# bharatlytics/faceRecognition_InfrenceEngine

Measured on AMD Instinct MI355X. Metric: faces/sec end-to-end @1080p, higher is better.
Workload: dtype f16

## Files before the change

### facerecognition_infrenceengine_amd/_lib.py

```python
import ctypes as C
import struct
import os
import threading

_HERE = os.path.dirname(os.path.abspath(__file__))
LIB_PATH = os.path.join(_HERE, "csrc", "libfrhip.so")

_lock = threading.Lock()
_lib = None
ABI_VERSION = 106


class FrError(RuntimeError):
    pass


class ConvArgs(C.Structure):
    _fields_ = [("x", C.c_void_p), ("w", C.c_void_p), ("y", C.c_void_p),
                ("bias", C.c_void_p), ("slope", C.c_void_p), ("residual", C.c_void_p),
                ("out_f32_partial", C.c_void_p),
                ("B", C.c_int), ("H", C.c_int), ("W", C.c_int), ("Cin", C.c_int), ("Cout", C.c_int),
                ("KH", C.c_int), ("KW", C.c_int), ("stride", C.c_int), ("pad", C.c_int),
                ("Ho", C.c_int), ("Wo", C.c_int), ("bias_mode", C.c_int), ("splitk", C.c_int),
                ("x2", C.c_void_p), ("C2", C.c_int)]
# ... 6 lines not shown
class ConvF8Args(C.Structure):
    _fields_ = [("x8", C.c_void_p), ("w8", C.c_void_p), ("y16", C.c_void_p), ("y8", C.c_void_p),
                ("oscale", C.c_void_p), ("bias", C.c_void_p), ("slope", C.c_void_p), ("residual", C.c_void_p),
                ("B", C.c_int), ("H", C.c_int), ("W", C.c_int), ("Cin", C.c_int), ("Cout", C.c_int),
                ("bias_mode", C.c_int), ("y8_mul", C.c_float), ("y8_sub", C.c_void_p)]


class RolePtr(C.c_void_p):
    role = None


class PnetLevel(C.Structure):
    _fields_ = [("x1", C.c_void_p), ("head", C.c_void_p), ("workspace", C.c_void_p), ("H1", C.c_int), ("W1", C.c_int),
                ("scale", C.c_float), ("boxes", C.c_void_p), ("scores", C.c_void_p), ("regs", C.c_void_p),
                ("counts", C.c_void_p), ("block_counts", C.c_void_p),
                ("x1s", C.c_void_p), ("hs", C.c_int), ("ws", C.c_int), ("f16", C.c_int)]


class FrameRef(C.Structure):
    _fields_ = [("data", C.c_void_p), ("H", C.c_int32), ("W", C.c_int32), ("nh", C.c_int32), ("nw", C.c_int32),
                ("reserved", C.c_int32 * 2)]


class Call(C.Structure):
    _fields_ = [("fn", C.c_int32), ("nargs", C.c_int32), ("a", C.c_uint64 * 22)]


_P, _I, _L, _F, _Z = C.c_void_p, C.c_int, C.c_int64, C.c_float, C.c_size_t
SEQ_FN = {"fr_dconv_mfma_f32": 1, "fr_pnet23_split_f16": 2, "fr_pnet_candidates": 3, "fr_sort_nms": 4, "fr_box_refine": 5,
          "fr_crop_conv1_f32": 6, "fr_stage_select": 7}

SIGNATURES = {
    "fr_version": (_I, []),
    "fr_last_error_string": (C.c_char_p, []),
    "fr_device_count": (_I, []),
    "fr_l2norm_rows_f32": (_I, [_P, _P, _I, _I, _P]),
    "fr_gallery_match_workspace": (_Z, [_I, _L]),
    "fr_gallery_match_f32": (_I, [_P, _P, _I, _L, _I, _L, _P, _P, _P, _Z, _P, _I, _P]),
    "fr_gallery_match_view_f32": (_I, [_P, _P, _P, _I, _L, _I, _P, _P, _P, _Z, _P]),
    "fr_gallery_topk_workspace": (_Z, [_I, _L, _I]),
    "fr_gallery_topk_f32": (_I, [_P, _P, _I, _L, _I, _I, _L, _P, _P, _P, _Z, _P, _I, _P]),
    "fr_gallery_topk_view_f32": (_I, [_P, _P, _P, _I, _L, _I, _I, _P, _P, _P, _Z, _P]),
    "fr_gallery_update_rows_f32": (_I, [_P, _P, _P, _I, _I, _I, _P]),
    "fr_gallery_match_f16_workspace": (_Z, [_I, _L]),
    "fr_gallery_match_f16": (_I, [_P, _P, _P, _I, _L, _I, _L, _P, _P, _P, _Z, _P, _I, _P]),
    "fr_gallery_match_f8_workspace": (_Z, [_I, _L]),
    "fr_gallery_match_f8": (_I, [_P, _P, _P, _I, _L, _I, _L, _P, _P, _P, _Z, _P, _I, _P]),
    "fr_gallery_update_rows_shadow": (_I, [_P, _P, _I, _P, _P, _I, _I, _I, _P]),
    "fr_gallery_match_view_f16_workspace": (_Z, [_I, _L]),
    "fr_gallery_match_view_f16": (_I, [_P, _P, _P, _P, _I, _L, _L, _I, _P, _P, _P, _Z, _P]),
    "fr_gallery_match_view_f8_workspace": (_Z, [_I, _L]),
    "fr_gallery_match_view_f8": (_I, [_P, _P, _P, _P, _I, _L, _L, _I, _P, _P, _P, _Z, _P]),
    "fr_gallery_topk_f16_workspace": (_Z, [_I, _L, _I]),
    "fr_gallery_topk_f16": (_I, [_P, _P, _P, _I, _L, _I, _I, _L, _P, _P, _P, _P, _P, _Z, _P, _I, _P]),
    "fr_gallery_topk_view_f16_workspace": (_Z, [_I, _L, _I]),
    "fr_gallery_topk_view_f16": (_I, [_P, _P, _P, _P, _I, _L, _L, _I, _I, _P, _P, _P, _P, _P, _Z, _P]),
    "fr_gallery_topk_view_masked_f32": (_I, [_P, _P, _P, _I, _L, _I, _I, _P, _P, _P, _Z, _P, _P]),
    "fr_gallery_match_grouped_workspace": (_Z, [_I, _L]),
    "fr_gallery_match_grouped_f32": (_I, [_P, _P, _P, _P, _P, _I, _I, _L, _L, _I, _P, _P, _P, _Z, _P, _I, _P]),
    "fr_gallery_topk_grouped_workspace": (_Z, [_I, _L, _I]),
    "fr_gallery_topk_grouped_f32": (_I, [_P, _P, _P, _P, _P, _I, _I, _L, _L, _I, _I, _P, _P, _P, _Z, _P, _I, _P]),
    "fr_gallery_gmax_update": (_I, [_P, _P, _L, _I, _P, _P]),
    "fr_f32_to_f8": (_I, [_P, _P, _L, _P]),
    "fr_f32_to_f16": (_I, [_P, _P, _L, _P]),
    "fr_match_decide": (_I, [_P, _P, _I, _F, _F, _P, _P]),
    "fr_match_pack_candidates": (_I, [_P, _P, _I, _P, _P]),
    "fr_match_reduce_shards": (_I, [_P, _I, _I, _I, _I, _P, _P, _P]),
    "fr_match_reduce_shards_topk": (_I, [_P, _I, _I, _I, _I, _I, _P, _P, _P]),
    "fr_exchange_pack_queries": (_I, [_P, _I, _I, _I, _P, _P]),
    "fr_exchange_counts": (_I, [_P, _I, _I, _I, _P, _P]),
    "fr_gallery_first_above_f32": (_I, [_P, _P, _I, _L, _I, _F, _I, _L, _P, _P, _P, _Z, _P]),
    "fr_cosine_matrix_f32": (_I, [_P, _P, _I, _I, _I, _P, _P]),
    "fr_mean_rows_f32": (_I, [_P, _I, _I, _P, _P]),
    "fr_unknown_assign_batch_f32": (_I, [_P, _P, _I, _I, _F, _P, _P, _P, _I, _I, _P, _P, _P, _P]),
    "fr_gallery_first_above_blocked_f32": (_I, [_P, _P, _P, _P, _I, _L, _I, _F, _I, _L, _P, _P, _P, _Z, _P]),
    "fr_enrol_batch_workspace": (_Z, [_I, _L]),
    "fr_enrol_batch_f32": (_I, [_P, _P, _I, _P, _P, _I, _P, _I, _I, _I, _P, _P, _L, _F, _F, _P, _P, _P, _P, _P, _P, _P, _P,
                                _Z, _P]),
    "fr_gallery_pairs_workspace": (_Z, [_L, _L]),
    "fr_gallery_pairs_above_f16": (_I, [_P, _P, _L, _I, _F, _I, _L, _I, _P, _P, _P, _P, _Z, _P]),
    "fr_conv_nhwc_f16": (_I, [C.POINTER(ConvArgs), _P]),
    "fr_conv_sequence": (_I, [C.POINTER(ConvStep), _I, _P]),
    "fr_conv_inblock_f16": (_I, [C.POINTER(ConvArgs), _P]),
    "fr_conv_nhwc_f8": (_I, [C.POINTER(ConvF8Args), _P]),
    "fr_quantize_f16_f8": (_I, [_P, _P, _L, _F, _P]),
    "fr_quantize_f16_f8_centred": (_I, [_P, _P, _L, _I, _P, _F, _P]),
    "fr_gptq_round_e4m3": (_I, [_P, _P, _P, _P, _I, _I, _P]),
    "fr_conv_stage14_weight_bytes": (_Z, [_I]),
    "fr_conv_stage14_pack": (_I, [_P, _P, _P]),
    "fr_conv_stage14_f16": (_I, [_P, _P, _P, _P, _I, _I, _P]),
    "fr_conv_walk64_weight_bytes": (_Z, [_I]),
    "fr_conv_walk64_pack": (_I, [_P, _P, _I, _P]),
    "fr_conv_walk64_f16": (_I, [_P, _P, _P, _P, _I, _P, _P, _I, _I, _I, _P]),
    "fr_conv_stage28_weight_bytes": (_Z, [_I]),
    "fr_conv_stage28_pack": (_I, [_P, _P, _P]),
    "fr_conv_stage28_f16": (_I, [_P, _P, _P, _P, _I, _I, _P]),
    "fr_conv_stage14_f8_weight_bytes": (_Z, [_I]),
    "fr_conv_stage14_f8_param_floats": (_Z, []),
    "fr_conv_stage14_f8_pack": (_I, [_P, _P, _P]),
    "fr_conv_stage14_f8": (_I, [_P, _P, _P, _P, _P, _I, _I, _P]),
    "fr_conv_splitk_epilogue": (_I, [_P, _I, _I, _I, _I, _I, _P, _I, _P, _P, _P, _P]),
    "fr_fc_reduce_l2norm": (_I, [_P, _I, _I, _I, _P, _P, _P, _P]),
    "fr_warp_affine_5pt": (_I, [_P, _I, _I, _I, _P, _P, _P, _I, _I, _P, _P, _P, _P]),
    "fr_warp_affine_5pt_slots": (_I, [_P, _I, _I, _I, _P, _P, _I, _I, _P, _P]),
    "fr_warp_affine_5pt_refs": (_I, [_P, _I, _P, _P, _P, _I, _I, _P, _P, _P, _P]),
    "fr_warp_affine_5pt_slots_refs": (_I, [_P, _I, _P, _P, _I, _I, _P, _P]),
    "fr_letterbox_u8": (_I, [_P, _I, _P, _I, _I, _P]),
    "fr_detections_unscale": (_I, [_P, _P, _P, _P, _I, _I, _P]),
    "fr_pyramid_resize_norm": (_I, [_P, _I, _I, _I, _I, _I, _P, _P]),
    "fr_dconv_f32": (_I, [_P, _P, _P, _P, _P, _I, _I, _I, _I, _I, _I, _I, _I, _I, _P, _P, _I, _P]),
    "fr_dconv_mfma_f32": (_I, [_I, _P, _P, _P, _P, _P, _I, _I, _I, _P, _P, _P, _I, _I, _P, _I, _P, _P]),
    "fr_crop_conv1_f32": (_I, [_I, _P, _I, _I, _I, _P, _P, _I, _P, _P, _P, _P, _P]),
    "fr_crop_conv1_split": (_I, [_I, _P, _I, _I, _I, _P, _P, _I, _P, _P, _P, _P, _I, _P]),
    "fr_crop_conv1_list_f32": (_I, [_I, _P, _I, _I, _I, _P, _I, _P, _P, _I, _P, _P, _P, _P, _P]),
    "fr_ro_conv2_split": (_I, [_I, _P, _P, _P, _P, _P, _I, _P, _I, _P, _P]),
    "fr_ro_gemm_weight_bytes": (_Z, [_I]),
    "fr_ro_gemm_pack": (_I, [_I, _P, _P, _P]),
    "fr_ro_gemm_split": (_I, [_I, _P, _P, _P, _P, _P, _I, _P, _I, _P]),
    "fr_ro_margin_list": (_I, [_P, _I, _P, _I, _I, _F, _F, _P, _P, _I, _P]),
    "fr_ro_scatter_rows": (_I, [_P, _P, _P, _I, _I, _P, _P]),
    "fr_pnet23_workspace_bytes": (_Z, [_I, _I, _I]),
    "fr_pnet23_split_f16": (_I, [_P, _P, _I, _I, _I, _P, _P, _P, _P, _P, _P, _P, _P, _P, _I, _F, _F, _P, _P, _Z, _P]),
    "fr_maxpool_f32": (_I, [_P, _P, _I, _I, _I, _I, _I, _I, _P]),
    "fr_pnet_conv1_band": (_I, [_I, _P, _I, _I, _I, _I, _I, _P, _P, _P, _P, _P, _P, _P, _I, _P]),
    "fr_pnet_band_tiles_count": (_Z, [_I, _I, _I]),
    "fr_pnet_band_tiles": (_I, [_P, _I, _I, _I, _P, _P, _P]),
    "fr_pnet_finish_levels": (_I, [C.POINTER(PnetLevel), _I, _I, _P, _P, _P, _P, _P, _P, _P, _P, _F, _I, _F, _P, _P]),
    "fr_pnet_pyramid_conv1": (_I, [_I, _P, _I, _I, _I, C.POINTER(PnetLevel), _I, _P, _P, _P, _P, _P, _I, _P]),
    "fr_pnet_pyramid_p23": (_I, [C.POINTER(PnetLevel), _I, _I, _P, _P, _P, _P, _P, _P, _P, _P, _I, _F, _F, _P]),
    "fr_pnet_pyramid_band_tiles": (_I, [C.POINTER(PnetLevel), _I, _I, _P, _P, _P]),
    "fr_pnet_candidates": (_I, [_P, _I, _I, _I, _F, _F, _I, _P, _P, _P, _P, _P, _P, _P, _F, _P]),
    "fr_sort_nms": (_I, [_P, _P, _P, _I, _P, _I, _I, _I, _I, _F, _I, _I, _P, _P, _P, _P, _I, _P]),
    "fr_box_refine": (_I, [_P, _P, _I, _P, _I, _I, _I, _P]),
    "fr_crop_resize_norm": (_I, [_P, _I, _I, _I, _P, _P, _I, _I, _P, _P]),
    "fr_stage_select": (_I, [_P, _P, _I, _P, _I, _I, _F, _P, _P, _P, _I, _P, _P, _P]),
    "fr_detect_sequence": (_I, [C.POINTER(Call), _I]),
    "fr_det_conv_weight_halves": (_Z, [_I, _I, _I]),
    "fr_det_conv_f16": (_I, [_P, _P, _P, _P, _P, _I, _I, _I, _I, _I, _I, _I, _I, _I, _I, _I, _I, _I, _I, _I, _P]),
    "fr_det_conv_act_f16": (_I, [_P, _P, _P, _P, _P, _P, _I, _I, _I, _I, _I, _I, _I, _I, _I, _I, _I, _I, _I, _I, _I, _P]),
    "fr_dw_conv_f16": (_I, [_P, _P, _P, _P, _P, _I, _I, _I, _I, _I, _I, _I, _I, _I, _I, _P]),
    "fr_det_input_f16": (_I, [_P, _P, _I, _I, _I, _P]),
    "fr_det_pool_f16": (_I, [_P, _P, _I, _I, _I, _I, _I, _I, _I, _I, _I, _I, _P]),
    "fr_det_upsample_add_f16": (_I, [_P, _P, _P, _I, _I, _I, _I, _I, _P]),
    "fr_scrfd_decode": (_I, [_P, _P, _P, _I, _I, _I, _I, _I, _I, _F, _P, _I, _P, _P, _P, _P, _P]),
}

_NOCHECK = ("fr_version", "fr_device_count")


def _slot(v, t):
    if t is _F:
        return struct.unpack("<I", struct.pack("<f", float(v)))[0]
    if t is _P:
        if v is None:
            return 0
        return int(v.value or 0) if isinstance(v, C.c_void_p) else int(v)
    return int(v) & 0xFFFFFFFFFFFFFFFF


class Lib:

    def __init__(self, cdll):
        self._c = cdll
        self._calls = {}
        self._rec = threading.local()
        for name, (res, args) in SIGNATURES.items():
            fn = getattr(cdll, name)
            fn.restype = res
            fn.argtypes = args
            if res is _I and name not in _NOCHECK:
                self._calls[name] = self._checked(name, fn)
            else:
                self._calls[name] = fn

    def _checked(self, name, fn):
        err = self._c.fr_last_error_string

        fid, types, rec = SEQ_FN.get(name), fn.argtypes, self._rec

        def call(*a):
            rc = fn(*a)
            if rc != 0:
                raise FrError(f"{name} failed ({rc}): {err().decode()}")
            if getattr(rec, "calls", None) is not None:
                rec.invalid = name
            return rc

        def call_rec(*a):
            rc = fn(*a)
            if rc != 0:
                raise FrError(f"{name} failed ({rc}): {err().decode()}")
            calls = getattr(rec, "calls", None)
            if calls is not None:
                calls.append((fid, [_slot(v, t) for v, t in zip(a, types)],
                              [(i, v.role) for i, v in enumerate(a) if isinstance(v, RolePtr)]))
            return rc
        return call_rec if fid is not None else call

    def start_recording(self):
        self._rec.calls, self._rec.invalid = [], None

    def note(self, fid, *slots):
        calls = getattr(self._rec, "calls", None)
        if calls is not None:
            calls.append((fid, [int(v.value or 0) if isinstance(v, C.c_void_p) else int(v) for v in slots], []))

    def stop_recording(self):
        calls, self._rec.calls = getattr(self._rec, "calls", None), None
        self._rec.last_invalid = getattr(self._rec, "invalid", None)
        self._rec.invalid = None
        return None if self._rec.last_invalid else calls

    def recording_invalid(self):
        return getattr(self._rec, "last_invalid", None)

    def __getattr__(self, name):
        try:
            return self.__dict__["_calls"][name]
        except KeyError:
            raise AttributeError(name)


def load():
    global _lib
    with _lock:
        if _lib is None:
            import torch
            if not os.path.exists(LIB_PATH):
                raise FrError(f"{LIB_PATH} not built: run `python -c 'import __graft_entry__ as g; g.build()'` "
                              f"or `make -C {os.path.dirname(LIB_PATH)}`; there is no CPU fallback")
# ... 29 lines not shown
```

### facerecognition_infrenceengine_amd/csrc/conv_mfma.hip

```cpp
#include "common.h"

#define BK 64

struct ConvP {
    const half_t* x; const half_t* w; half_t* y;
    const float* bias; const float* slope; const half_t* res; float* partial;
    int B, H, W, Cin, Cout, KH, KW, stride, pad, Ho, Wo, bias_mode, splitk;
    int M, K, nk;
    unsigned xbytes, wbytes;
    const half_t* x2; int C2, nk_main; unsigned x2bytes;
};

template <int WN>
__device__ __forceinline__ void conv_epilogue(const ConvP& p, float4v (&acc)[4][4], int cout0, int m0, int wc, int wp,
                                              int fr, int fq) {
    const int HoWo = p.Ho * p.Wo;
#pragma unroll
    for (int j = 0; j < 4; ++j) {
        const int m = m0 + wp * 64 + j * 16 + fr;
        if (m >= p.M) continue;
        int bsel = 0;
        if (p.bias_mode == 1) {
            int r = m % HoWo;
            int ho = r / p.Wo, wo = r - ho * p.Wo;
// ... 94 lines not shown
        int kh, kw, tapoff;
        if (SMALL_CIN) {
            int tap = s * 8 + tchunk;
            kh = tap / p.KW; kw = tap - kh * p.KW;
            if (tap >= p.KH * p.KW) kh = 1 << 14;
            tapoff = (kh * p.W + kw) * p.Cin * 2;
        } else {
            int tap = s / cin_steps, c0 = (s - tap * cin_steps) * BK;
            kh = tap / p.KW; kw = tap - kh * p.KW;
            tapoff = ((kh * p.W + kw) * p.Cin + c0) * 2;
        }
        half_t* wl = lds + buf * (BN + BM) * BK;
        half_t* xl = wl + BN * BK;
#pragma unroll
        for (int i = 0; i < WROWS; ++i)
            __builtin_amdgcn_raw_ptr_buffer_load_lds(wrs, (lds_ptr_t)(wl + (wave * WROWS + i) * 8 * BK), 16,
                                                     wbase[i] + (unsigned)s * (BK * 2), 0, 0, 0);
        if (!SMALL_CIN && s >= p.nk_main) {
#pragma unroll
            for (int i = 0; i < XROWS; ++i)
                __builtin_amdgcn_raw_ptr_buffer_load_lds(x2rs, (lds_ptr_t)(xl + (wave * XROWS + i) * 8 * BK), 16,
                                                         x2off(i, (s - p.nk_main) * BK), 0, 0, 0);
            return;
        }
#pragma unroll
        for (int i = 0; i < XROWS; ++i) {
            int hi = (xhw[i] >> 16) + kh, wi = (int)(short)(xhw[i] & 0xffff) + kw;
            bool ok = (unsigned)hi < (unsigned)p.H && (unsigned)wi < (unsigned)p.W;
            unsigned off = ok ? (unsigned)(xbase[i] + tapoff) : 0x80000000u;
            __builtin_amdgcn_raw_ptr_buffer_load_lds(xrs, (lds_ptr_t)(xl + (wave * XROWS + i) * 8 * BK), 16, off, 0, 0, 0);
        }
    };

    float4v acc[4][4];
#pragma unroll
    for (int i = 0; i < 4; ++i)
#pragma unroll
        for (int j = 0; j < 4; ++j) acc[i][j] = float4v{0.f, 0.f, 0.f, 0.f};

    const int fr = lane & 15, fq = lane >> 4;
    if (ks < ke) {
        gload_lds(ks, 0);
        asm volatile("s_waitcnt vmcnt(0)" ::: "memory");
    }
    __syncthreads();
    for (int s = ks; s < ke; ++s) {
        const int buf = (s - ks) & 1;
        if (s + 1 < ke) gload_lds(s + 1, buf ^ 1);
        const half_t* wl = lds + buf * (BN + BM) * BK + (wc * 64) * BK;
        const half_t* xl = lds + buf * (BN + BM) * BK + BN * BK + (wp * 64) * BK;
#pragma unroll
        for (int kk = 0; kk < 2; ++kk) {
            half8 a[4], b[4];
            const int ch = kk * 4 + fq;
#pragma unroll
            for (int i = 0; i < 4; ++i) {
                int row = i * 16 + fr;
                a[i] = *reinterpret_cast<const half8*>(wl + row * BK + ((ch ^ (row & 7)) << 3));
                b[i] = *reinterpret_cast<const half8*>(xl + row * BK + ((ch ^ (row & 7)) << 3));
            }
#pragma unroll
            for (int i = 0; i < 4; ++i)
#pragma unroll
                for (int j = 0; j < 4; ++j)
                    acc[i][j] = __builtin_amdgcn_mfma_f32_16x16x32_f16(a[i], b[j], acc[i][j], 0, 0, 0);
        }
        asm volatile("s_waitcnt vmcnt(0)" ::: "memory");
        __syncthreads();
    }

    conv_epilogue<WN>(p, acc, cout0, m0, wc, wp, fr, fq);
#endif
}

template <int WN, bool SMALL>
static void launch_conv(const ConvP& p, hipStream_t s) {
    constexpr int BN = 64 * WN, BM = 64 * (4 / WN);
    dim3 grid((p.M + BM - 1) / BM, p.Cout / BN, p.splitk > 1 ? p.splitk : 1);
    conv_mfma_kernel<WN, SMALL><<<grid, 256, 0, s>>>(p);
}

int fr_conv_halo_try(const fr_conv_args* a, hipStream_t s);
int fr_conv_stem_try(const fr_conv_args* a, hipStream_t s);

extern "C" int fr_conv_nhwc_f16(const fr_conv_args* a, fr_stream_t stream) {
    FR_REQUIRE(a, "fr_conv_nhwc_f16: null args");
    FR_REQUIRE(a->x && a->w && (a->y || a->out_f32_partial), "fr_conv_nhwc_f16: null tensor");
    FR_REQUIRE(a->B > 0 && a->H > 0 && a->W > 0 && a->KH > 0 && a->KW > 0 && a->stride > 0 && a->pad >= 0,
               "fr_conv_nhwc_f16: bad geometry");
    FR_REQUIRE(a->Ho == (a->H + 2 * a->pad - a->KH) / a->stride + 1 && a->Wo == (a->W + 2 * a->pad - a->KW) / a->stride + 1,
               "fr_conv_nhwc_f16: Ho/Wo do not match the geometry");
    FR_REQUIRE(a->Cout % 64 == 0, "fr_conv_nhwc_f16: Cout must be a multiple of 64 (got %d)", a->Cout);
    const bool small = a->Cin == 8;
    FR_REQUIRE(small || a->Cin % 64 == 0, "fr_conv_nhwc_f16: Cin must be 8 or a multiple of 64 (got %d)", a->Cin);
    FR_REQUIRE(a->bias_mode == 0 || (a->bias_mode == 1 && a->KH == 3 && a->KW == 3 && a->stride == 1 && a->pad == 1 &&
                                     a->Ho >= 2 && a->Wo >= 2),
               "fr_conv_nhwc_f16: bias_mode 1 needs a 3x3/s1/p1 conv");
    FR_REQUIRE(a->H < 32768 && a->W < 32768, "fr_conv_nhwc_f16: H/W too large");
    ConvP p;
    p.x = (const half_t*)a->x; p.w = (const half_t*)a->w; p.y = (half_t*)a->y;
    p.bias = a->bias; p.slope = a->slope; p.res = (const half_t*)a->residual; p.partial = a->out_f32_partial;
    p.B = a->B; p.H = a->H; p.W = a->W; p.Cin = a->Cin; p.Cout = a->Cout; p.KH = a->KH; p.KW = a->KW;
    p.stride = a->stride; p.pad = a->pad; p.Ho = a->Ho; p.Wo = a->Wo; p.bias_mode = a->bias_mode;
    p.splitk = a->splitk > 1 ? a->splitk : 1;
    FR_REQUIRE(p.splitk == 1 || p.partial, "fr_conv_nhwc_f16: splitk > 1 needs out_f32_partial");
    int64_t M = (int64_t)a->B * a->Ho * a->Wo;
    int64_t xbytes = (int64_t)a->B * a->H * a->W * a->Cin * 2;
    int Kreal = a->KH * a->KW * a->Cin;
    FR_REQUIRE(!a->x2 || (!small && a->C2 > 0 && a->C2 % 64 == 0 && (a->H - 1) / a->stride + 1 >= a->Ho && (a->W - 1) / a->stride + 1 >= a->Wo),
               "fr_conv_nhwc_f16: x2 needs Cin %% 64 == 0, C2 %% 64 == 0 and every (ho * stride, wo * stride) inside the image");
    p.x2 = (const half_t*)a->x2; p.C2 = a->x2 ? a->C2 : 0;
    p.K = small ? ((Kreal + 127) / 128) * 128 : Kreal + p.C2;
    p.nk_main = Kreal / BK;
    int64_t x2bytes = (int64_t)a->B * a->H * a->W * p.C2 * 2;
    FR_REQUIRE(x2bytes < (1ll << 31), "fr_conv_nhwc_f16: x2 too large for 32-bit buffer offsets");
    p.x2bytes = (unsigned)x2bytes;
    int64_t wbytes = (int64_t)a->Cout * p.K * 2;
    FR_REQUIRE(M < (1ll << 31) && xbytes < (1ll << 31) && wbytes < (1ll << 31) && M * a->Cout * 2 < (1ll << 40),
               "fr_conv_nhwc_f16: tensor too large for 32-bit buffer offsets (split the batch)");
    p.M = (int)M; p.nk = p.K / BK; p.xbytes = (unsigned)xbytes; p.wbytes = (unsigned)wbytes;
    hipStream_t s = fr_stream(stream);
    const int h = fr_conv_halo_try(a, s);
    if (h < 0) return h;
    if (h == 1) {
        FR_CHECK_LAUNCH("conv_halo_kernel");
        return FR_OK;
    }
    if (small) {
        if (fr_conv_stem_try(a, s) == 1) {
            FR_CHECK_LAUNCH("conv_stem_kernel");
            return FR_OK;
        }
    }
    if (small) {
        if (a->Cout % 128 == 0) launch_conv<2, true>(p, s); else launch_conv<1, true>(p, s);
    } else if (a->Cout % 128 == 0) {
        launch_conv<2, false>(p, s);
    } else {
        launch_conv<1, false>(p, s);
    }
    FR_CHECK_LAUNCH("conv_mfma_kernel");
    return FR_OK;
}

__global__ void conv_splitk_epilogue(const float* __restrict__ partial, int splitk, int M, int Cout, int Ho, int Wo,
                                     const float* __restrict__ bias, int bias_mode, const float* __restrict__ slope,
                                     const half_t* __restrict__ res, half_t* __restrict__ y) {
    const int q4 = Cout / 4;
    const int64_t e = (int64_t)blockIdx.x * blockDim.x + threadIdx.x;
    if (e >= (int64_t)M * q4) return;
    const int m = (int)(e / q4), co = (int)(e - (int64_t)m * q4) * 4;
    float4v v = {0.f, 0.f, 0.f, 0.f};
    for (int z = 0; z < splitk; ++z) v += *reinterpret_cast<const float4v*>(partial + ((size_t)z * M + m) * Cout + co);
    if (bias) {
        int bsel = 0;
        if (bias_mode == 1) {
            const int r = m % (Ho * Wo), ho = r / Wo, wo = r - ho * Wo;
            const int rc = ho == 0 ? 0 : (ho == Ho - 1 ? 2 : 1), cc = wo == 0 ? 0 : (wo == Wo - 1 ? 2 : 1);
            bsel = (rc * 3 + cc) * Cout;
        }
        v += *reinterpret_cast<const float4v*>(bias + bsel + co);
    }
    if (slope) {
        const float4v sv = *reinterpret_cast<const float4v*>(slope + co);
#pragma unroll
        for (int c = 0; c < 4; ++c) v[c] = v[c] > 0.f ? v[c] : v[c] * sv[c];
    }
    if (res) {
        const half4 rv = *reinterpret_cast<const half4*>(res + (size_t)m * Cout + co);
#pragma unroll
        for (int c = 0; c < 4; ++c) v[c] += (float)rv[c];
    }
    *reinterpret_cast<half4*>(y + (size_t)m * Cout + co) = half4{(half_t)v[0], (half_t)v[1], (half_t)v[2], (half_t)v[3]};
}

extern "C" int fr_conv_splitk_epilogue(const float* partial, int splitk, int M, int Cout, int Ho, int Wo,
                                       const float* bias, int bias_mode, const float* slope, const void* residual,
                                       void* y, fr_stream_t stream) {
    FR_REQUIRE(partial && y && splitk >= 1 && M > 0 && Cout > 0 && Cout % 4 == 0 && Ho > 0 && Wo > 0,
               "fr_conv_splitk_epilogue: bad argument");
    FR_REQUIRE(bias_mode == 0 || (bias_mode == 1 && bias && Ho >= 2 && Wo >= 2), "fr_conv_splitk_epilogue: bad bias mode");
    const int64_t n = (int64_t)M * (Cout / 4);
    conv_splitk_epilogue<<<(unsigned)((n + 255) / 256), 256, 0, fr_stream(stream)>>>(
        partial, splitk, M, Cout, Ho, Wo, bias, bias_mode, slope, (const half_t*)residual, (half_t*)y);
    FR_CHECK_LAUNCH("conv_splitk_epilogue");
    return FR_OK;
}

extern "C" int fr_conv_sequence(const fr_conv_step* steps, int nsteps, fr_stream_t stream) {
    FR_REQUIRE(steps && nsteps > 0, "fr_conv_sequence: no steps");
    for (int i = 0; i < nsteps; ++i) {
        const fr_conv_step& st = steps[i];
        int rc;
        if (st.kind == 0) {
            rc = fr_conv_nhwc_f16(&st.args, stream);
        } else if (st.kind == 1) {
            const fr_conv_args& a = st.args;
            FR_REQUIRE(a.splitk > 1 && a.out_f32_partial && a.y, "fr_conv_sequence: step %d: split-K step without splitk / partial / y", i);
            fr_conv_args p = a;
            p.y = nullptr; p.bias = nullptr; p.slope = nullptr; p.residual = nullptr; p.bias_mode = 0;
            rc = fr_conv_nhwc_f16(&p, stream);
            if (rc == FR_OK)
                rc = fr_conv_splitk_epilogue(a.out_f32_partial, a.splitk, a.B * a.Ho * a.Wo, a.Cout, a.Ho, a.Wo, a.bias,
                                             a.bias_mode, a.slope, a.residual, a.y, stream);
        } else if (st.kind == 2) {
            rc = fr_conv_inblock_f16(&st.args, stream);
        } else {
            FR_REQUIRE(false, "fr_conv_sequence: step %d: unknown kind %d", i, st.kind);
        }
        if (rc != FR_OK) return rc;
// ... 61 lines not shown
```

### include/frhip.h

```cpp
#ifndef FRHIP_H
#define FRHIP_H
#include <stddef.h>
#include <stdint.h>
#ifdef __cplusplus
extern "C" {
#endif

#define FR_OK 0
#define FR_E_INVALID (-1)
#define FR_E_LAUNCH (-2)
#define FR_E_NODEVICE (-3)

typedef void* fr_stream_t;

#define FR_ABI_VERSION 106
int fr_version(void);
const char* fr_last_error_string(void);
int fr_device_count(void);

int fr_l2norm_rows_f32(const float* x, float* out, int rows, int dim, fr_stream_t stream);

size_t fr_gallery_match_workspace(int F, int64_t N);
int fr_gallery_match_f32(const float* Q, const float* G, int F, int64_t N, int D,
                         int64_t row_offset, int64_t* out_idx, float* out_score,
// ... 72 lines not shown
                           float* out_score, fr_stream_t stream);
int fr_match_reduce_shards_topk(const int32_t* cand_all, int R, int n, int K, int q0, int F,
                                int64_t* out_idx, float* out_score, fr_stream_t stream);
int fr_exchange_pack_queries(const float* Q, int F, int q_max, int D, float* send, fr_stream_t stream);
int fr_exchange_counts(const float* gathered, int R, int q_max, int D, int32_t* counts, fr_stream_t stream);


int fr_gallery_first_above_f32(const float* Q, const float* G, int F, int64_t N, int D, float thr,
                               int inclusive, int64_t row_offset, int64_t* out_idx, float* out_score,
                               void* workspace, size_t workspace_bytes, fr_stream_t stream);
int fr_cosine_matrix_f32(const float* A, const float* B, int F, int N, int D, float* out,
                         fr_stream_t stream);
int fr_mean_rows_f32(const float* x, int K, int D, float* out, fr_stream_t stream);
#define FR_UNKNOWN_N 0
#define FR_UNKNOWN_OVERFLOW 1
#define FR_UNKNOWN_HEADER 4
#define FR_UNKNOWN_STATE_INTS(capacity) (FR_UNKNOWN_HEADER + 3 * (capacity))
int fr_unknown_assign_batch_f32(const float* E, const int32_t* take, int F, int D, float thr, float* avg, float* hist,
                                int32_t* state, int capacity, int depth, int32_t* out_cluster, int32_t* out_new,
                                int32_t* out_count, fr_stream_t stream);

int fr_gallery_first_above_blocked_f32(const float* Q, const float* G, const int64_t* view, const int32_t* take, int F,
                                       int64_t N, int D, float thr, int inclusive, int64_t row_offset, int64_t* out_idx,
                                       float* out_score, void* workspace, size_t workspace_bytes, fr_stream_t stream);
#define FR_ENROL_DONE 0
#define FR_ENROL_NO_FACE 1
#define FR_ENROL_DIFFERENT 2
#define FR_ENROL_DUPLICATE 3
#define FR_ENROL_MAX_POSES 8
#define FR_ENROL_MAX_JOBS 256
size_t fr_enrol_batch_workspace(int J, int64_t N);
int fr_enrol_batch_f32(const float* E, const float* bbox, int S, const int32_t* img_first, const int32_t* img_count, int I,
                       const int32_t* job_first, int J, int max_poses, int D, const float* G, const int64_t* view, int64_t N,
                       float sim_thr, float dup_thr, int32_t* status, int32_t* pair, int32_t* face, float* avg, float* row,
                       int64_t* dup_pos, float* dup_score, void* workspace, size_t workspace_bytes, fr_stream_t stream);
#define FR_PAIRS_OVERFLOW 1
#define FR_PAIRS_NONFINITE 2
size_t fr_gallery_pairs_workspace(int64_t N, int64_t capacity);
int fr_gallery_pairs_above_f16(const float* G32, const int64_t* view, int64_t N, int D, float thr, int inclusive,
                               int64_t capacity, int max_ranges, int64_t* out_key, float* out_score, int32_t* out_counts,
                               void* workspace, size_t workspace_bytes, fr_stream_t stream);

typedef struct {
    const void* x; const void* w; void* y;
    const float* bias; const float* slope; const void* residual;
    float* out_f32_partial;
    int B, H, W, Cin, Cout, KH, KW, stride, pad, Ho, Wo;
    int bias_mode; int splitk;
    const void* x2; int C2;
} fr_conv_args;
int fr_conv_nhwc_f16(const fr_conv_args* args, fr_stream_t stream);
typedef struct {
    const void* x8; const void* w8; void* y16; void* y8;
    const float* oscale; const float* bias; const float* slope; const void* residual;
    int B, H, W, Cin, Cout, bias_mode;
    float y8_mul;
    const float* y8_sub;
} fr_conv_f8_args;
int fr_conv_nhwc_f8(const fr_conv_f8_args* args, fr_stream_t stream);
int fr_quantize_f16_f8(const void* x16, void* out8, int64_t n, float mul, fr_stream_t stream);
int fr_quantize_f16_f8_centred(const void* x16, void* out8, int64_t n, int C, const float* sub, float mul,
                               fr_stream_t stream);
size_t fr_conv_stage14_weight_bytes(int nconv);
int fr_conv_stage14_pack(const void* w, void* out, fr_stream_t stream);
int fr_conv_stage14_f16(const void* x, void* y, const void* wstream, const float* params, int B, int nblocks,
                        fr_stream_t stream);
size_t fr_conv_stage28_weight_bytes(int nconv);
int fr_conv_stage28_pack(const void* w, void* out, fr_stream_t stream);
int fr_conv_stage28_f16(void* x, void* mid, const void* wstream, const float* params, int B, int nblocks, fr_stream_t stream);
size_t fr_conv_walk64_weight_bytes(int Cout);
int fr_conv_walk64_pack(const void* w, void* out, int Cout, fr_stream_t stream);
int fr_conv_walk64_f16(const void* x, const void* wstream, void* y, const float* bias, int bias_mode, const float* slope,
                       const void* residual, int B, int HW, int Cout, fr_stream_t stream);
size_t fr_conv_stage14_f8_weight_bytes(int nconv);
size_t fr_conv_stage14_f8_param_floats(void);
int fr_conv_stage14_f8_pack(const void* w8, void* out, fr_stream_t stream);
int fr_conv_stage14_f8(const void* x8, const void* x16, void* y16, const void* wstream, const float* params, int B,
                       int nblocks, fr_stream_t stream);
int fr_gptq_round_e4m3(const double* W, const double* U, const float* sw, float* Q, int rows, int K, fr_stream_t stream);
int fr_conv_splitk_epilogue(const float* partial, int splitk, int M, int Cout, int Ho, int Wo,
                            const float* bias, int bias_mode, const float* slope, const void* residual,
                            void* y, fr_stream_t stream);
int fr_conv_inblock_f16(const fr_conv_args* args, fr_stream_t stream);
typedef struct {
    int kind;
    fr_conv_args args;
} fr_conv_step;
int fr_conv_sequence(const fr_conv_step* steps, int nsteps, fr_stream_t stream);
int fr_fc_reduce_l2norm(const float* partial, int splitk, int B, int dim, const float* bias,
                        float* embedding, float* normed, fr_stream_t stream);


int fr_warp_affine_5pt(const uint8_t* frames, int nframes, int H, int W, const float* kps,
                       const int32_t* frame_idx, const int32_t* count, int F, int size,
                       void* out_f16_nhwc8, uint8_t* out_u8_bgr, float* M_out, fr_stream_t stream);

int fr_warp_affine_5pt_slots(const uint8_t* frames, int nframes, int H, int W, const float* kps,
                             const int32_t* counts, int cap, int size, void* out_f16_nhwc8,
                             fr_stream_t stream);

typedef struct {
    const uint8_t* data;
    int32_t H, W, nh, nw;
    int32_t reserved[2];
} fr_frame_ref;
int fr_warp_affine_5pt_refs(const fr_frame_ref* refs, int nframes, const float* kps, const int32_t* frame_idx,
                            const int32_t* count, int F, int size, void* out_f16_nhwc8, uint8_t* out_u8_bgr,
                            float* M_out, fr_stream_t stream);
int fr_warp_affine_5pt_slots_refs(const fr_frame_ref* refs, int nframes, const float* kps, const int32_t* counts,
                                  int cap, int size, void* out_f16_nhwc8, fr_stream_t stream);

int fr_pyramid_resize_norm(const uint8_t* frames, int nframes, int H, int W, int hs, int ws,
                           float* out, fr_stream_t stream);
int fr_dconv_f32(const float* x, const float* w, const float* bias, const float* slope, float* y,
                 int B, int H, int W, int Cin, int Cout, int CoutP, int KH, int KW, int pool2,
                 const float* head_w, const float* head_b, int nhead, fr_stream_t stream);
int fr_dconv_mfma_f32(int layer, const float* x, const float* w, const float* bias, const float* slope,
                      float* y, int B, int H, int W, const float* head_w, const float* head_b,
                      const uint8_t* frames, int FH, int FW, const int32_t* counts, int cap, void* y_split,
                      fr_stream_t stream);
int fr_crop_conv1_f32(int net, const uint8_t* frames, int nframes, int H, int W, const float* boxes,
                      const int32_t* counts, int cap, const float* w, const float* bias, const float* slope,
                      float* y, fr_stream_t stream);
int fr_crop_conv1_split(int net, const uint8_t* frames, int nframes, int H, int W, const float* boxes,
                        const int32_t* counts, int cap, const float* w, const float* bias, const float* slope,
                        void* y_split, int conv_f16, fr_stream_t stream);
int fr_crop_conv1_list_f32(int net, const uint8_t* frames, int nframes, int H, int W, const float* boxes, int cap,
                           const int32_t* list, const int32_t* list_count, int list_cap, const float* w,
                           const float* bias, const float* slope, float* y, fr_stream_t stream);
int fr_ro_conv2_split(int net, const void* x_split, const float* w, const float* bias, const float* slope, float* y,
                      int nslots, const int32_t* counts, int cap, int32_t* zero_word, fr_stream_t stream);
size_t fr_ro_gemm_weight_bytes(int layer);
int fr_ro_gemm_pack(int layer, const float* w, void* out, fr_stream_t stream);
int fr_ro_gemm_split(int layer, const float* x, const void* w_packed, const float* bias, const float* slope, float* y,
                     int nslots, const int32_t* counts, int cap, fr_stream_t stream);
int fr_ro_margin_list(const float* head, int nhead, const int32_t* counts, int nframes, int cap, float logit_thr,
                      float margin, int32_t* list, int32_t* list_count, int list_cap, fr_stream_t stream);
int fr_ro_scatter_rows(const float* src, const int32_t* list, const int32_t* list_count, int list_cap, int ncols,
                       float* dst, fr_stream_t stream);
size_t fr_pnet23_workspace_bytes(int B, int H1, int W1);
int fr_pnet23_split_f16(const float* x1, const void* x1s, int B, int H1, int W1, const float* w2, const float* b2, const float* s2,
                        const float* w3, const float* b3, const float* s3, const float* hw, const float* hb,
                        float* head, int all_heads, float refine_logit_thr, float refine_band_hi, int32_t* refined_count,
                        void* workspace, size_t workspace_bytes, fr_stream_t stream);
int fr_maxpool_f32(const float* x, float* y, int B, int H, int W, int C, int k, int stride,
                   fr_stream_t stream);
int fr_pnet_candidates(const float* head, int nframes, int hc, int wc, float scale, float thr, int cap,
                       float* boxes, float* scores, float* regs, int32_t* counts,
                       int32_t* block_counts, float* prob_out, const float* dl, float dl_min, fr_stream_t stream);
int fr_sort_nms(const float* boxes, const float* scores, const float* aux, int naux,
                const int32_t* counts, int L, int nseg, int seg_cap, int seg_major, float thr, int mode,
                int max_keep,
                float* boxes_out, float* scores_out, float* aux_out, int32_t* counts_out,
                int cap_out, fr_stream_t stream);
int fr_box_refine(float* boxes, const float* aux, int naux, const int32_t* counts, int L, int cap,
                  int mode, fr_stream_t stream);
int fr_crop_resize_norm(const uint8_t* frames, int nframes, int H, int W, const float* boxes,
                        const int32_t* counts, int cap, int size, float* out, fr_stream_t stream);
int fr_stage_select(const float* boxes, const float* head, int nh, const int32_t* counts, int L, int cap,
                    float thr, float* boxes_out, float* scores_out, float* aux_out, int naux,
                    int32_t* counts_out, float* prob_out, fr_stream_t stream);

int fr_pnet_conv1_band(int mode, const uint8_t* frames, int B, int FH, int FW, int H, int W, const float* w, const float* bias,
                       const float* slope, float* y, void* y_split, const int32_t* list, const int32_t* list_count, int list_cap,
                       fr_stream_t stream);
size_t fr_pnet_band_tiles_count(int B, int H1, int W1);
// ... 56 lines not shown
```

Baseline: 25990.

## Add dedicated 3x3 stride-2 entry conv kernel with fused shortcut and LDS pipelining

Adds a specialised MFMA kernel for the 3x3/stride-2/pad-1 stage-entry convolutions, optionally fusing a second input (the shortcut operand x2) as an extra K phase. It loads directly into LDS through buffer loads with a multi-stage ring, uses 512-thread workgroups with large pixel tiles and Cout-dependent tile widths, and fuses bias, PReLU and residual in the epilogue. It runs ahead of the generic path only when the grid would have enough tiles. The trade-off is higher LDS and register pressure and more code paths to tune.

```diff
diff --git a/facerecognition_infrenceengine_amd/_lib.py b/facerecognition_infrenceengine_amd/_lib.py
--- a/facerecognition_infrenceengine_amd/_lib.py
+++ b/facerecognition_infrenceengine_amd/_lib.py
@@ -112,6 +112,8 @@
     "fr_conv_nhwc_f16": (_I, [C.POINTER(ConvArgs), _P]),
     "fr_conv_sequence": (_I, [C.POINTER(ConvStep), _I, _P]),
     "fr_conv_inblock_f16": (_I, [C.POINTER(ConvArgs), _P]),
+    "fr_conv_entry_f16": (_I, [C.POINTER(ConvArgs), _I, _P]),
+    "fr_conv_entry_min_tiles": (_I, [_I]),
     "fr_conv_nhwc_f8": (_I, [C.POINTER(ConvF8Args), _P]),
     "fr_quantize_f16_f8": (_I, [_P, _P, _L, _F, _P]),
     "fr_quantize_f16_f8_centred": (_I, [_P, _P, _L, _I, _P, _F, _P]),
@@ -175,7 +177,7 @@
     "fr_scrfd_decode": (_I, [_P, _P, _P, _I, _I, _I, _I, _I, _I, _F, _P, _I, _P, _P, _P, _P, _P]),
 }
 
-_NOCHECK = ("fr_version", "fr_device_count")
+_NOCHECK = ("fr_version", "fr_device_count", "fr_conv_entry_min_tiles")
 
 
 def _slot(v, t):
diff --git a/facerecognition_infrenceengine_amd/csrc/conv_entry.hip b/facerecognition_infrenceengine_amd/csrc/conv_entry.hip
--- /dev/null
+++ b/facerecognition_infrenceengine_amd/csrc/conv_entry.hip
@@ -0,0 +1,268 @@
+#include "common.h"
+#include <type_traits>
+
+namespace {
+
+constexpr int EN_PX = 196;
+constexpr int EN_NPT = 13;
+constexpr int EN_WIDE = 392;
+constexpr int EN_MIN_WGS = 256;
+
+struct EntryP {
+    const half_t* x; const half_t* w; half_t* y;
+    const float* bias; const float* slope; const half_t* res; const half_t* x2;
+    int H, W, Cin, Cout, Ho, Wo, C2;
+    int M, K, nk;
+    unsigned xbytes, wbytes, x2bytes;
+};
+
+}
+
+template <int BN, int NPT, int NS, int MINW>
+__global__ __launch_bounds__(512, MINW) void conv_entry_kernel(EntryP p) {
+#if defined(__HIP_DEVICE_COMPILE__)
+    constexpr int WN = BN / 64, WP = 8 / WN;
+    constexpr int NPW = BN / 16;
+    constexpr int PX = EN_PX * ((NPT + EN_NPT - 1) / EN_NPT);
+    constexpr int NP = NPW + NPT;
+    constexpr int DMAX = (NP + 7) / 8, DMIN = NP / 8;
+    constexpr int SLOT = NP * 1024;
+    constexpr unsigned OOB = 0x80000000u;
+    extern __shared__ __attribute__((aligned(16))) char lds[];
+
+    const int tid = threadIdx.x, lane = tid & 63;
+    const int wave = __builtin_amdgcn_readfirstlane(tid >> 6);
+    const int wn = wave % WN, wp = wave / WN;
+    const int fr = lane & 15, fq = lane >> 4;
+    const int m0 = blockIdx.x * PX, cout0 = blockIdx.y * BN;
+
+    __amdgpu_buffer_rsrc_t xrs = buffer_rsrc(p.x, p.xbytes);
+    __amdgpu_buffer_rsrc_t wrs = buffer_rsrc(p.w, p.wbytes);
+    __amdgpu_buffer_rsrc_t x2rs = buffer_rsrc(p.x2 ? p.x2 : p.x, p.x2 ? p.x2bytes : 0u);
+
+    const int prow = lane >> 2;
+    const int schunk = (lane & 3) ^ (((lane >> 5) & 1) << 1);
+    int base1[DMAX], base2[DMAX], pmask[DMAX];
+    const int HoWo = p.Ho * p.Wo;
+#pragma unroll
+    for (int k = 0; k < DMAX; ++k) {
+        const int pc = wave + 8 * k;
+        base1[k] = base2[k] = 0; pmask[k] = 0;
+        if (pc < NPW) {
+            base1[k] = base2[k] = ((cout0 + pc * 16 + prow) * p.K + schunk * 8) * 2;
+            pmask[k] = 0x3ff;
+        } else if (pc < NP) {
+            const int row = (pc - NPW) * 16 + prow, m = m0 + row;
+            if (row < PX && m < p.M) {
+                const int n = m / HoWo, r = m - n * HoWo;
+                const int ho = r / p.Wo, wo = r - ho * p.Wo;
+                const int bh = ho * 2 - 1, bw = wo * 2 - 1;
+                base1[k] = (((n * p.H + bh) * p.W + bw) * p.Cin + schunk * 8) * 2;
+                base2[k] = (((n * p.H + bh + 1) * p.W + bw + 1) * p.C2 + schunk * 8) * 2;
+                int mk = 1 << 9;
+#pragma unroll
+                for (int t = 0; t < 9; ++t)
+                    if ((unsigned)(bh + t / 3) < (unsigned)p.H && (unsigned)(bw + t % 3) < (unsigned)p.W) mk |= 1 << t;
+                pmask[k] = mk;
+            }
+        }
+    }
+
+    int i_q = 0, i_tap = 0, i_kw = 0, i_c = 0, i_tapbase = 0;
+    const int cin2 = p.Cin * 2;
+    auto issue = [&](int slotoff) {
+        const bool ph2 = i_tap >= 9;
+        const int bit = i_q >= p.nk ? 10 : (ph2 ? 9 : i_tap);
+        const int soffx = ph2 ? i_c : i_tapbase + i_c;
+        const int soffw = i_q * 64;
+#pragma unroll
+        for (int k = 0; k < DMAX; ++k) {
+            const int pc = wave + 8 * k;
+            if (k >= DMIN && pc >= NP) continue;
+            char* dst = lds + slotoff + pc * 1024;
+            const bool ok = (pmask[k] >> bit) & 1;
+            if (pc < NPW) {
+                __builtin_amdgcn_raw_ptr_buffer_load_lds(wrs, (lds_ptr_t)dst, 16, ok ? (unsigned)(base1[k] + soffw) : OOB, 0, 0, 0);
+            } else if (ph2) {
+                __builtin_amdgcn_raw_ptr_buffer_load_lds(x2rs, (lds_ptr_t)dst, 16, ok ? (unsigned)(base2[k] + soffx) : OOB, 0, 0, 0);
+            } else {
+                __builtin_amdgcn_raw_ptr_buffer_load_lds(xrs, (lds_ptr_t)dst, 16, ok ? (unsigned)(base1[k] + soffx) : OOB, 0, 0, 0);
+            }
+        }
+        ++i_q; i_c += 64;
+        if (!ph2 && i_c == cin2) {
+            i_c = 0; ++i_tap; ++i_kw; i_tapbase += cin2;
+            if (i_kw == 3) { i_kw = 0; i_tapbase += (p.W - 3) * cin2; }
+        }
+    };
+
+#pragma unroll
+    for (int i = 0; i < NS; ++i) issue(i * SLOT);
+
+    auto run = [&](auto wp_tag) {
+        constexpr int WPI = decltype(wp_tag)::value;
+        constexpr int PT = NPT / WP + (WPI < NPT % WP ? 1 : 0);
+        constexpr int T0 = WPI * (NPT / WP) + (WPI < NPT % WP ? WPI : NPT % WP);
+        constexpr bool EARLY = WPI * WN < 4;
+        constexpr int NR = 4 + PT;
+        constexpr int RPG = (NR + PT - 1) / PT;
+        constexpr int JMID = PT / 2;
+
+        const int f_lane = fr * 64 + ((fq ^ (((fr >> 3) & 1) << 1)) << 4);
+        const int a_off = wn * 4096 + f_lane, b_off = (NPW + T0) * 1024 + f_lane;
+        float4v acc[4][PT];
+#pragma unroll
+        for (int i = 0; i < 4; ++i)
+#pragma unroll
+            for (int j = 0; j < PT; ++j) acc[i][j] = float4v{0.f, 0.f, 0.f, 0.f};
+        int4v a0[4], b0[PT], a1[4], b1[PT];
+
+        auto rd = [&](int4v (&a)[4], int4v (&b)[PT], int slotoff, int r) {
+            if (r < 4) a[r] = *reinterpret_cast<const int4v*>(lds + slotoff + a_off + r * 1024);
+            else if (r < NR) b[r - 4] = *reinterpret_cast<const int4v*>(lds + slotoff + b_off + (r - 4) * 1024);
+        };
+        auto step = [&](int4v (&ac)[4], int4v (&bc)[PT], int4v (&an)[4], int4v (&bn)[PT], int s_free, int s_next) {
+            if constexpr (EARLY) { issue(s_free); FR_PIN(); }
+#pragma unroll
+            for (int j = 0; j < PT; ++j) {
+#pragma unroll
+                for (int r = j * RPG; r < (j + 1) * RPG; ++r) rd(an, bn, s_next, r);
+#pragma unroll
+                for (int i = 0; i < 4; ++i) acc[i][j] = mfma16(ac[i], bc[j], acc[i][j]);
+                FR_PIN();
+                if constexpr (!EARLY) { if (j == JMID) { issue(s_free); FR_PIN(); } }
+            }
+        };
+
+        asm volatile("s_waitcnt vmcnt(%0)" ::"n"((NS - 1) * DMIN) : "memory");
+        __builtin_amdgcn_s_barrier();
+#pragma unroll
+        for (int r = 0; r < NR; ++r) rd(a0, b0, 0, r);
+        auto after = [](int slot) { return slot + SLOT == NS * SLOT ? 0 : slot + SLOT; };
+        int s_cur = 0;
+#pragma unroll 1
+        for (int s = 0; s < p.nk; s += 2) {
+            asm volatile("s_waitcnt vmcnt(%0) lgkmcnt(0)" ::"n"((NS - 2) * DMIN) : "memory");
+            __builtin_amdgcn_s_barrier();
+            FR_PIN();
+            int s_next = after(s_cur);
+            step(a0, b0, a1, b1, s_cur, s_next);
+            asm volatile("s_waitcnt vmcnt(%0) lgkmcnt(0)" ::"n"((NS - 2) * DMIN) : "memory");
+            __builtin_amdgcn_s_barrier();
+            FR_PIN();
+            s_cur = s_next; s_next = after(s_cur);
+            step(a1, b1, a0, b0, s_cur, s_next);
+            s_cur = s_next;
+        }
+        asm volatile("s_waitcnt vmcnt(0) lgkmcnt(0)" ::: "memory");
+
+#pragma unroll
+        for (int j = 0; j < PT; ++j) {
+            const int row = (T0 + j) * 16 + fr, m = m0 + row;
+            if (row >= PX || m >= p.M) continue;
+#pragma unroll
+            for (int i = 0; i < 4; ++i) {
+                const int co = cout0 + wn * 64 + i * 16 + fq * 4;
+                float4v v = acc[i][j];
+                if (p.bias) {
+                    float4v bv = *reinterpret_cast<const float4v*>(p.bias + co);
+                    v += bv;
+                }
+                if (p.slope) {
+                    float4v sv = *reinterpret_cast<const float4v*>(p.slope + co);
+#pragma unroll
+                    for (int e = 0; e < 4; ++e) v[e] = v[e] > 0.f ? v[e] : v[e] * sv[e];
+                }
+                const size_t o = (size_t)m * p.Cout + co;
+                if (p.res) {
+                    half4 rv = *reinterpret_cast<const half4*>(p.res + o);
+#pragma unroll
+                    for (int e = 0; e < 4; ++e) v[e] += (float)rv[e];
+                }
+                half4 hv = {(half_t)v[0], (half_t)v[1], (half_t)v[2], (half_t)v[3]};
+                *reinterpret_cast<half4*>(p.y + o) = hv;
+            }
+        }
+    };
+    static_for<WP>([&](auto t) {
+        if (wp == decltype(t)::value) run(t);
+    });
+#endif
+}
+
+template <int BN, int NPT, int NS, int MINW>
+static int launch_entry(const EntryP& p, hipStream_t s) {
+    constexpr size_t lds = (size_t)NS * (BN / 16 + NPT) * 1024;
+    constexpr int PX = EN_PX * ((NPT + EN_NPT - 1) / EN_NPT);
+    static FrDevLatch latch;
+    auto kern = conv_entry_kernel<BN, NPT, NS, MINW>;
+    if (!fr_raise_lds(reinterpret_cast<const void*>(kern), lds, latch)) {
+        fr_set_error("conv_entry: cannot raise dynamic LDS to %zu bytes", lds);
+        return FR_E_LAUNCH;
+    }
+    dim3 grid((p.M + PX - 1) / PX, p.Cout / BN);
+    kern<<<grid, 512, lds, s>>>(p);
+    return FR_OK;
+}
+
+static bool entry_shape(const fr_conv_args* a, EntryP& p) {
+    if (!a || !a->x || !a->w || !a->y || a->out_f32_partial) return false;
+    if (!(a->KH == 3 && a->KW == 3 && a->stride == 2 && a->pad == 1 && a->bias_mode == 0 && a->splitk <= 1)) return false;
+    if (a->B <= 0 || a->H <= 0 || a->W <= 0 || a->H >= 32768 || a->W >= 32768) return false;
+    if (a->Ho != (a->H - 1) / 2 + 1 || a->Wo != (a->W - 1) / 2 + 1) return false;
+    if (a->Cin <= 0 || a->Cin % 64 != 0 || a->Cout <= 0 || a->Cout % 64 != 0) return false;
+    if (a->x2 && (a->C2 <= 0 || a->C2 % 64 != 0)) return false;
+    const int C2 = a->x2 ? a->C2 : 0;
+    const int64_t M = (int64_t)a->B * a->Ho * a->Wo, K = 9ll * a->Cin + C2;
+    const int64_t xbytes = (int64_t)a->B * a->H * a->W * a->Cin * 2, x2bytes = (int64_t)a->B * a->H * a->W * C2 * 2;
+    const int64_t wbytes = (int64_t)a->Cout * K * 2;
+    if (M + EN_PX >= (1ll << 31) || xbytes >= (1ll << 31) || x2bytes >= (1ll << 31) || wbytes >= (1ll << 31) ||
+        M * a->Cout * 2 >= (1ll << 40))
+        return false;
+    p.x = (const half_t*)a->x; p.w = (const half_t*)a->w; p.y = (half_t*)a->y;
+    p.bias = a->bias; p.slope = a->slope; p.res = (const half_t*)a->residual; p.x2 = (const half_t*)a->x2;
+    p.H = a->H; p.W = a->W; p.Cin = a->Cin; p.Cout = a->Cout; p.Ho = a->Ho; p.Wo = a->Wo; p.C2 = C2;
+    p.M = (int)M; p.K = (int)K; p.nk = (int)(K / 32);
+    p.xbytes = (unsigned)xbytes; p.wbytes = (unsigned)wbytes; p.x2bytes = (unsigned)x2bytes;
+    return true;
+}
+
+static int entry_bn(int Cout) { return Cout % 128 != 0 ? 64 : (Cout == 256 ? 256 : 128); }
+static int entry_min_tiles(int Cout) {
+    const int groups = Cout / entry_bn(Cout);
+    return (EN_MIN_WGS + groups - 1) / groups;
+}
+
+static int entry_launch(const EntryP& p, int form, hipStream_t s) {
+    if (form == 0) {
+        const int64_t tiles = ((int64_t)p.M + EN_PX - 1) / EN_PX;
+        form = entry_bn(p.Cout);
+        if (form == 128 && (tiles / 2) * (p.Cout / 128) >= EN_MIN_WGS) form = EN_WIDE;
+    }
+    if (form == EN_WIDE) return launch_entry<128, 25, 3, 2>(p, s);
+    if (form == 256) return launch_entry<256, 13, 4, 2>(p, s);
+    if (form == 128) return launch_entry<128, 13, 5, 2>(p, s);
+    return launch_entry<64, 13, 4, 4>(p, s);
+}
+
+int fr_conv_entry_try(const fr_conv_args* a, hipStream_t s) {
+    EntryP p;
+    if (!entry_shape(a, p)) return 0;
+    if ((p.M + EN_PX - 1) / EN_PX < entry_min_tiles(p.Cout)) return 0;
+    const int rc = entry_launch(p, 0, s);
+    return rc == FR_OK ? 1 : rc;
+}
+
+extern "C" int fr_conv_entry_min_tiles(int Cout) { return Cout > 0 && Cout % 64 == 0 ? entry_min_tiles(Cout) : 0; }
+
+extern "C" int fr_conv_entry_f16(const fr_conv_args* a, int bn, fr_stream_t stream) {
+    EntryP p;
+    FR_REQUIRE(entry_shape(a, p), "fr_conv_entry_f16: a 3x3 / stride 2 / pad 1 conv with Cin, Cout (and C2) multiples of 64, a plain bias, "
+                                  "a fused epilogue and no split-K");
+    FR_REQUIRE(bn == 0 || ((bn == 64 || bn == 128 || bn == 256) && p.Cout % bn == 0) || (bn == EN_WIDE && p.Cout % 128 == 0),
+               "fr_conv_entry_f16: bn must be 0, 64, 128, 256 or 392 and its couts divide Cout (got %d, Cout %d)", bn, p.Cout);
+    const int rc = entry_launch(p, bn, fr_stream(stream));
+    if (rc != FR_OK) return rc;
+    FR_CHECK_LAUNCH("conv_entry_kernel");
+    return FR_OK;
+}
diff --git a/facerecognition_infrenceengine_amd/csrc/conv_mfma.hip b/facerecognition_infrenceengine_amd/csrc/conv_mfma.hip
--- a/facerecognition_infrenceengine_amd/csrc/conv_mfma.hip
+++ b/facerecognition_infrenceengine_amd/csrc/conv_mfma.hip
@@ -200,6 +200,7 @@
 
 int fr_conv_halo_try(const fr_conv_args* a, hipStream_t s);
 int fr_conv_stem_try(const fr_conv_args* a, hipStream_t s);
+int fr_conv_entry_try(const fr_conv_args* a, hipStream_t s);
 
 extern "C" int fr_conv_nhwc_f16(const fr_conv_args* a, fr_stream_t stream) {
     FR_REQUIRE(a, "fr_conv_nhwc_f16: null args");
@@ -244,6 +245,12 @@
         FR_CHECK_LAUNCH("conv_halo_kernel");
         return FR_OK;
     }
+    const int e = fr_conv_entry_try(a, s);
+    if (e < 0) return e;
+    if (e == 1) {
+        FR_CHECK_LAUNCH("conv_entry_kernel");
+        return FR_OK;
+    }
     if (small) {
         if (fr_conv_stem_try(a, s) == 1) {
             FR_CHECK_LAUNCH("conv_stem_kernel");
diff --git a/include/frhip.h b/include/frhip.h
--- a/include/frhip.h
+++ b/include/frhip.h
@@ -178,6 +178,8 @@
                             const float* bias, int bias_mode, const float* slope, const void* residual,
                             void* y, fr_stream_t stream);
 int fr_conv_inblock_f16(const fr_conv_args* args, fr_stream_t stream);
+int fr_conv_entry_f16(const fr_conv_args* args, int bn, fr_stream_t stream);
+int fr_conv_entry_min_tiles(int Cout);
 typedef struct {
     int kind;
     fr_conv_args args;
```

Result: slower. 25220 (-3.0%).
